# mdangschat/ctc-asr

Measured on AMD Instinct MI355X. Metric: audio-seconds/s training throughput (DS2, 10 s utterances), higher is better.
Workload: dtype f32 tensors / accumulate / own kernels; projection GEMMs: fp16x3 split (22 significand bits) where the layer input is bounded or, behind a ReLU cell, scaled per row / per column on the device - forward projections and their gradient GEMMs - bf16x6 split (24 bits) elsewhere; forward and backward recu

## Files before the change

ctc_asr_amd/csrc/rnn_persistent.hip:

```cpp
#include "common.h"
#include <stddef.h>
#include <stdlib.h>
#include <string.h>
#include <type_traits>
#include <vector>

#define PRNN_THREADS 256
#define PRNN_BLOCK_ROWS 32
#ifndef PRNN_GROUPS
#define PRNN_GROUPS 8
#endif
#define PRNN_SPIN_LIMIT (1u << 22)
#ifndef PRNN_PROBE_RS_Q
#define PRNN_PROBE_RS_Q 4
#endif
#ifndef PRNN_PROBE_HALF_LOADS
#define PRNN_PROBE_HALF_LOADS 0
#endif
#ifndef PRNN_XCD_AWARE
#define PRNN_XCD_AWARE 0
#endif
#ifndef PRNN_CHAIN_LB
#define PRNN_CHAIN_LB 4
#endif
// ... 41 lines not shown
    const float *b_hh;
    float *drec;
    float *dbias;
    int T, B, H, nwg;
    int BS;
    int ndir, dir0;
    int chain0;
    int s_lo, s_hi;
    float *carry;
    float *rs;
    unsigned *colmax;
    int prof;
    unsigned ticket;
    int xcd_split;
    unsigned *kp;
};

__device__ __forceinline__ float4 ldg4(const float *p) {
    return *reinterpret_cast<const float4 *>(p);
}
__device__ __forceinline__ void mma4(f32x4 &acc, const float4 &a, const float4 &b) {
    acc = __builtin_amdgcn_mfma_f32_16x16x4f32(a.x, b.x, acc, 0, 0, 0);
    acc = __builtin_amdgcn_mfma_f32_16x16x4f32(a.y, b.y, acc, 0, 0, 0);
    acc = __builtin_amdgcn_mfma_f32_16x16x4f32(a.z, b.z, acc, 0, 0, 0);
    acc = __builtin_amdgcn_mfma_f32_16x16x4f32(a.w, b.w, acc, 0, 0, 0);
}
__device__ __forceinline__ void mma4x2(f32x4 &acc0, f32x4 &acc1, const float4 &a0,
                                       const float4 &b0, const float4 &a1, const float4 &b1) {
    acc0 = __builtin_amdgcn_mfma_f32_16x16x4f32(a0.x, b0.x, acc0, 0, 0, 0);
    acc1 = __builtin_amdgcn_mfma_f32_16x16x4f32(a1.x, b1.x, acc1, 0, 0, 0);
// ... 482 lines not shown
                                         unsigned uniform_off) {
    return __builtin_amdgcn_raw_buffer_load_b128(rsrc, (int)lane_off, (int)uniform_off, 0);
}
template <int CTRL>
__device__ __forceinline__ unsigned dpp_u32(unsigned v) {
    return (unsigned)__builtin_amdgcn_update_dpp(0, (int)v, CTRL, 0xF, 0xF, false);
}
__device__ __forceinline__ void gather8_pieces(unsigned q0, u32x4 &first, u32x4 &second) {
    const unsigned q1 = dpp_u32<0x101>(q0), q2 = dpp_u32<0x102>(q0), q3 = dpp_u32<0x103>(q0),
                   q4 = dpp_u32<0x104>(q0), q5 = dpp_u32<0x105>(q0), q6 = dpp_u32<0x106>(q0),
                   q7 = dpp_u32<0x107>(q0);
    first = (u32x4){(q0 & 0xFFFFu) | (q1 << 16), (q2 & 0xFFFFu) | (q3 << 16),
                    (q4 & 0xFFFFu) | (q5 << 16), (q6 & 0xFFFFu) | (q7 << 16)};
    second = (u32x4){(q0 >> 16) | (q1 & 0xFFFF0000u), (q2 >> 16) | (q3 & 0xFFFF0000u),
                     (q4 >> 16) | (q5 & 0xFFFF0000u), (q6 >> 16) | (q7 & 0xFFFF0000u)};
}

template <int CELL, int NT, int KC, int REGW = 0>
__global__ void __launch_bounds__(PRNN_THREADS) prnn_fwd16_kernel(PArgs p) {
    constexpr bool GRU = CELL == CTCASR_CELL_GRU;
    constexpr int G = 4;
    constexpr int GR = GRU ? 3 : G;
    constexpr int COLS = 16 * NT;
    constexpr int UPB = COLS / G;
    constexpr int QS = KC * NT * 2;
    constexpr int QL = QS - REGW;
    constexpr int QW = 2 * KC;
    static_assert(16 * UPB <= PRNN_THREADS, "one item per thread");
    extern __shared__ __attribute__((aligned(16))) char smem[];
    resident_signal(p.sync, p.ticket);
// ... 1206 lines not shown
#ifndef PRNN_B16S_XCD_EXCL
#define PRNN_B16S_XCD_EXCL 0
#endif
#ifndef PRNN_B16S_JA
#define PRNN_B16S_JA 1
#endif
template <int DD, int JW, int JP, int JA, bool PROF = false>
__global__ void __launch_bounds__(PRNN_THREADS) prnn_bwd16s_kernel(PArgs p) {
    constexpr int H = PRNN_RS_H, GH = 4 * H;
    constexpr int NW = 4, NTH = 256, NPW = 16, QS = NPW * 4, QL = QS / 2, REGW = QS - QL;
    constexpr int RED_FLOATS = NW * 16 * 17, IVL = 4 * NPW;
    static_assert(DD % 2 == 0 && DD <= NPW && (NPW % DD == 0 || JW == NPW / 2 - 1),
                  "ring slots: even; not a divisor of 16 only when the next phase is requested at the end");
    static_assert(2 * JW >= NPW - DD && JW < NPW / 2 && JP <= JW && JA <= JP, "pipeline points");
    extern __shared__ __attribute__((aligned(16))) char smem[];
    resident_signal(p.sync, p.ticket);
    if (launch_poisoned(p.sync)) return;
    u32x4 *frag = reinterpret_cast<u32x4 *>(smem);
    float *red = reinterpret_cast<float *>(smem + (size_t)NW * QL * 64 * sizeof(u32x4));
    float4 *invs = reinterpret_cast<float4 *>(red + 2 * RED_FLOATS);
    float *wave_top = reinterpret_cast<float *>(invs + 2 * NW * IVL);
    unsigned *arrived = reinterpret_cast<unsigned *>(wave_top + 4);

    const int tid = threadIdx.x, lane = tid & 63;
    const int wave = __builtin_amdgcn_readfirstlane(tid >> 6);
#if PRNN_B16S_XCD_EXCL
    if (((int)blockIdx.x & 7) >= 4) return;
    const int dir = p.dir0 + (((int)blockIdx.x & 7) >> 1);
    const int slice = ((int)blockIdx.x >> 3) * 2 + ((int)blockIdx.x & 1);
#else
    const int wg = blockIdx.x % (p.ndir * p.nwg);
    const bool split = p.xcd_split && p.ndir == 2;
    const int dir = p.dir0 + (split ? (wg & 7) >> 2 : wg / p.nwg);
    const int slice = split ? (wg >> 3) * 4 + (wg & 3) : wg % p.nwg;
#endif
    const int group_size = p.nwg / PRNN_GROUPS, grp = slice / group_size;
    const int B = p.B, T = p.T, BS = p.BS;
    const int u0 = slice * 16;
    if (tid < 2) arrived[tid] = 0u;

    float w_scale;
    {
        float m = 0.f;
        const float *wrow = p.w + ((size_t)dir * H + u0 + (tid & 15)) * GH;
        for (int n = (tid >> 4) * 4; n < GH; n += NTH / 16 * 4) {
            const float4 v = ldg4(wrow + n);
            m = fmaxf(fmaxf(m, fmaxf(fabsf(v.x), fabsf(v.y))), fmaxf(fabsf(v.z), fabsf(v.w)));
        }
        m = wave_max(m);
        if (lane == 0) wave_top[wave] = m;
        __syncthreads();
        m = fmaxf(fmaxf(wave_top[0], wave_top[1]), fmaxf(wave_top[2], wave_top[3]));
        const unsigned bits = __float_as_uint(m);
        const int e = (int)((bits >> 23) & 0xFF) - 127;
        const int se = bits == 0u ? 0 : min(max(14 - e, -60), 60);
        w_scale = __uint_as_float((unsigned)(se + 127) << 23);
    }
    const float out_scale = 1.0f / w_scale;
    u32x4 wreg[REGW];
    {
        auto pieces = [&](int pm, u32x4 &first, u32x4 &second) {
            const float *wcol = p.w + ((size_t)dir * H + u0 + (lane & 15)) * GH +
                                16 * (wave * NPW + (pm >> 1)) + 8 * (pm & 1) + 2 * (lane >> 4);
            unsigned q[8];
#pragma unroll
            for (int e = 0; e < 8; ++e)
                q[e] = f16_pieces(wcol[(size_t)(e & 3) * H + (e >> 2)] * w_scale);
            first = (u32x4){(q[0] & 0xFFFFu) | (q[1] << 16), (q[2] & 0xFFFFu) | (q[3] << 16),
                            (q[4] & 0xFFFFu) | (q[5] << 16), (q[6] & 0xFFFFu) | (q[7] << 16)};
            second = (u32x4){(q[0] >> 16) | (q[1] & 0xFFFF0000u), (q[2] >> 16) | (q[3] & 0xFFFF0000u),
                             (q[4] >> 16) | (q[5] & 0xFFFF0000u), (q[6] >> 16) | (q[7] & 0xFFFF0000u)};
        };
        for (int pm = 0; pm < QL / 2; ++pm) {
            u32x4 first, second;
            pieces(pm, first, second);
            frag[(wave * QL + 2 * pm) * 64 + lane] = first;
            frag[(wave * QL + 2 * pm + 1) * 64 + lane] = second;
        }
#pragma unroll
        for (int pm = 0; pm < REGW / 2; ++pm) pieces(QL / 2 + pm, wreg[2 * pm], wreg[2 * pm + 1]);
    }
    __syncthreads();

    const __amdgpu_buffer_rsrc_t x_rsrc = __builtin_amdgcn_make_buffer_rsrc(
        p.xchg, 0, (int)((size_t)(T + 1) * 2 * B * GH * sizeof(float)), 0x00020000);
    const size_t x_step = (size_t)2 * B * GH;
    const size_t x_base = x_step;
    const __amdgpu_buffer_rsrc_t s_rsrc = __builtin_amdgcn_make_buffer_rsrc(
        p.rs, 0, (int)prnn_b16_scale_bytes(T), 0x00020000);
    constexpr unsigned S_STEP = 2u * (H / 16) * PRNN_B16_SCALE_ROWS * sizeof(float);
    const int rnum = 0x7FFFFFFF;
    const __amdgpu_buffer_rsrc_t dy_rsrc = __builtin_amdgcn_make_buffer_rsrc(
        const_cast<float *>(p.dy), 0, rnum, 0x00020000);
    const __amdgpu_buffer_rsrc_t g_rsrc = __builtin_amdgcn_make_buffer_rsrc(p.gates, 0, rnum, 0x00020000);
    const __amdgpu_buffer_rsrc_t c_rsrc = __builtin_amdgcn_make_buffer_rsrc(p.cells, 0, rnum, 0x00020000);
    const __amdgpu_buffer_rsrc_t dx_rsrc = __builtin_amdgcn_make_buffer_rsrc(p.dxw, 0, rnum, 0x00020000);
    auto ldf = [](__amdgpu_buffer_rsrc_t r, unsigned off) -> float {
// ... 1611 lines not shown
    }
    return CTCASR_ERR_BAD_ARGUMENT;
}

static size_t prnn_step_exchange_bytes(int T, int B, int H, int G) {
    return ctcasr_align_up((size_t)(T + 1) * 2 * B * G * H * sizeof(float), 256);
}
size_t prnn_exchange_bytes(int T, int B, int H, int G) {
    return prnn_step_exchange_bytes(T, B, H, G) +
           (G == 4 && H == PRNN_RS_H
                ? prnn_rs_ring_bytes() + ctcasr_align_up(prnn_b16_scale_bytes(T), 256) : 0) +
           (G == 4 && H == PRNN_W16_H ? ctcasr_align_up(prnn_w16_scale_bytes(T), 256) : 0) +
           (G == 1 && H == PRNN_R16_H ? prnn_r16_scale_bytes(T) : 0);
}

int prnn_fwd(int cell, const float *xw, const float *xw_bias, const float *w_hh,
             const float *b_hh_n, const int32_t *seq_len, int T, int B, int BS, int H, float *y,
             void *y16, float *gates, float *cells, void *sync, void *xchg, float *carry,
             int step_begin, int step_end, int flags, hipStream_t s) {
    const bool fwd_half_chip = (flags & CTCASR_RNN_HALF_CHIP) != 0;
    PArgs p = {};
    p.carry = carry;
    p.xchg = reinterpret_cast<float *>(xchg);
    p.xw = xw; p.w = w_hh; p.seq_len = seq_len; p.y = y; p.gates = gates; p.cells = cells;
    p.y16 = reinterpret_cast<unsigned short *>(y16);
    p.bias = xw_bias; p.b_hh = b_hh_n;
    p.ndir = 2; p.dir0 = 0; p.chain0 = 0;
    p.sync = reinterpret_cast<SyncWords *>(sync);
    p.T = T; p.B = B; p.BS = BS; p.H = H;
    p.s_lo = step_begin; p.s_hi = step_end;
// ... 78 lines not shown
        PRNN_FWD(CTCASR_CELL_LSTM, 2, 16, 2);
    }
    if (cell == CTCASR_CELL_RNN_RELU) {
        if (mt == 1) { PRNN_FWD(CTCASR_CELL_RNN_RELU, 1, 32, 1); }
        PRNN_FWD(CTCASR_CELL_RNN_RELU, 1, 32, 2);
    }
    if (mt == 1) { PRNN_FWD(CTCASR_CELL_RNN_TANH, 1, 32, 1); }
    PRNN_FWD(CTCASR_CELL_RNN_TANH, 1, 32, 2);
#undef PRNN_FWD
}

int prnn_bwd(int cell, const float *dy, const float *y, const float *w_hh_t,
             const int32_t *seq_len, int T, int B, int BS, int H, const float *gates,
             const float *cells, float *dxw, float *drec, float *dbias, unsigned *colmax,
             void *sync, void *kp, void *xchg, float *carry, int step_begin, int step_end,
             int flags, hipStream_t s) {
    PArgs p = {};
    p.dbias = dbias;
    p.s_lo = step_begin; p.s_hi = step_end; p.carry = carry;
    p.xchg = reinterpret_cast<float *>(xchg);
    p.w = w_hh_t; p.seq_len = seq_len; p.y = const_cast<float *>(y); p.dy = dy; p.dxw = dxw;
    p.drec = drec;
    p.gates = const_cast<float *>(gates); p.cells = const_cast<float *>(cells);
    p.sync = reinterpret_cast<SyncWords *>(sync);
    const bool half_chip = (flags & CTCASR_RNN_WHOLE_CHIP) == 0;
    p.T = T; p.B = B; p.BS = BS; p.H = H;
    p.ndir = 2; p.dir0 = 0; p.chain0 = 0;
    p.nwg = cell == CTCASR_CELL_LSTM ? (half_chip ? H / 16 : H / 8) : (half_chip ? H / 32 : H / 16);
    p.prof = getenv("CTCASR_RNN_PROF") != nullptr;
    p.ticket = ((unsigned)flags >> 8) & 0xFFFFFFu;
    p.xcd_split = (flags & CTCASR_RNN_XCD_SPLIT) != 0;
    const int mt = (B + 15) / 16;
    const bool chains = mt == 2 && !(flags & CTCASR_RNN_ONE_BARRIER);
// ... 187 lines not shown
```

ctc_asr_amd/csrc/rnn_step.hip:

```cpp
#include "common.h"

#define RNN_THREADS 256

namespace {

struct StepArgs {
    const float *xw;
    const float *w;
    const int *seq_len;
    float *y;
    const float *dy;
    float *dxw;
    float *gates;
    float *cells;
    float *hbuf;
    float *cbuf;
    const float *b_hh;
    const float *xw_bias;
    float *drec;
    int T, B, H, step;
};

__device__ __forceinline__ float4 ldg4(const float *p) {
    return *reinterpret_cast<const float4 *>(p);
// ... 227 lines not shown

extern "C" int ctcasr_rnn_persistent_supported(int cell, int T, int B, int H);
size_t prnn_sync_bytes();
size_t prnn_error_offset();
size_t prnn_kp_region_bytes(int H, int G);
int prnn_resident_gate(void *sync, unsigned ticket, int max_wait_us, hipStream_t s);
size_t prnn_exchange_bytes(int T, int B, int H, int G);
int prnn_fwd(int cell, const float *xw, const float *xw_bias, const float *w_hh,
             const float *b_hh_n, const int32_t *seq_len, int T, int B, int BS, int H, float *y,
             void *y16, float *gates, float *cells, void *sync, void *xchg, float *carry,
             int step_begin, int step_end, int flags, hipStream_t s);
int prnn_bwd(int cell, const float *dy, const float *y, const float *w_hh_t,
             const int32_t *seq_len, int T, int B, int BS, int H, const float *gates,
             const float *cells, float *dxw, float *drec, float *dbias, unsigned *colmax,
             void *sync, void *kp, void *xchg, float *carry, int step_begin, int step_end,
             int flags, hipStream_t s);

#define PRNN_BLOCK_ROWS 32
static int prnn_blocks(int B) { return (B + PRNN_BLOCK_ROWS - 1) / PRNN_BLOCK_ROWS; }
static int prnn_block_rows(int B, int block) {
    const int left = B - block * PRNN_BLOCK_ROWS;
    return left < PRNN_BLOCK_ROWS ? left : PRNN_BLOCK_ROWS;
}

static size_t rnn_state_bytes(int B, int H) {
    return ctcasr_align_up((size_t)6 * B * H * sizeof(float), 256);
}

static size_t prnn_ctl_bytes(int H, int G) {
    return ctcasr_align_up(prnn_sync_bytes(), 256) +
           ctcasr_align_up(prnn_kp_region_bytes(H, G), 256);
// ... 135 lines not shown
    const int rows = B < PRNN_BLOCK_ROWS ? B : PRNN_BLOCK_ROWS;
    return (flags & CTCASR_RNN_F16) &&
           ((cell == CTCASR_CELL_LSTM && (H == 1024 || H == 2048)) ||
            (cell == CTCASR_CELL_RNN_RELU && H == 2048 && rows <= 16 && B <= 16)) &&
           ctcasr_rnn_persistent_supported(cell, T, B, H) ? 1 : 0;
}

extern "C" int ctcasr_rnn_f16_recurrence(int cell, int T, int B, int H, int flags, int backward,
                                         int ragged) {
    if (cell == CTCASR_CELL_RNN_RELU)
        return !ragged && ctcasr_rnn_bwd_f16_supported(cell, T, B, H, flags);
    return backward ? ctcasr_rnn_bwd_f16_supported(cell, T, B, H, flags)
                    : ctcasr_rnn_fwd_f16_supported(cell, T, B, H, flags);
}

extern "C" int ctcasr_rnn_bwd_steps(int cell, const float *dy, const float *y,
                                    const float *w_hh_t, const float *b_hh_n,
                                    const int32_t *seq_len, int T, int B, int H,
                                    const void *reserve, float *dxw, float *dbias,
                                    uint32_t *colmax, void *workspace, size_t workspace_bytes,
                                    int step_begin, int step_end, int flags,
                                    ctcasr_stream_t stream) {
    (void)b_hh_n;
    if (colmax && (!ctcasr_rnn_bwd_f16_supported(cell, T, B, H, flags) ||
                   (cell == CTCASR_CELL_RNN_RELU && seq_len)))
        return CTCASR_ERR_UNSUPPORTED;
    int rc = rnn_check(cell, T, B, H);
    if (rc != CTCASR_OK) return rc;
    if (flags & 0xFF & ~(CTCASR_RNN_HALF_CHIP | CTCASR_RNN_WHOLE_CHIP | CTCASR_RNN_ONE_BARRIER |
                         CTCASR_RNN_REDUCE_SCATTER | CTCASR_RNN_F16 | CTCASR_RNN_XCD_SPLIT |
                         CTCASR_RNN_STAGGER | CTCASR_RNN_KPAIR))
        return CTCASR_ERR_BAD_ARGUMENT;
    if (!dy || !y || !w_hh_t || !reserve || !dxw) return CTCASR_ERR_BAD_ARGUMENT;
    if (step_begin < 0 || step_end > T || step_begin >= step_end) return CTCASR_ERR_BAD_ARGUMENT;
    if (!workspace || workspace_bytes < ctcasr_rnn_workspace_bytes(cell, T, B, H))
        return CTCASR_ERR_WORKSPACE;
    hipStream_t s = (hipStream_t)stream;
// ... 11 lines not shown
        return CTCASR_ERR_LAUNCH;
    if (cell == CTCASR_CELL_GRU && seq_len && step_end == T &&
        hipMemsetAsync(p.drec, 0, (size_t)T * B * 2 * G * H * sizeof(float), s) != hipSuccess)
        return CTCASR_ERR_LAUNCH;
    if (ctcasr_rnn_persistent_supported(cell, T, B, H)) {
        for (int blk = 0; blk < prnn_blocks(B); ++blk) {
            const size_t b0 = (size_t)blk * PRNN_BLOCK_ROWS;
            const PrnnBlock wb = prnn_block(workspace, T, B, H, G, blk);
            if (step_end == T &&
                (rc = prnn_clear_zero_block(wb, blk, prnn_block_rows(B, blk), H, G, s)) != CTCASR_OK)
                return rc;
            rc = prnn_bwd(cell, dy + b0 * 2 * H, y + b0 * 2 * H, w_hh_t,
                          seq_len ? seq_len + b0 : nullptr, T, prnn_block_rows(B, blk), B, H,
                          p.gates + b0 * 2 * 4 * H, p.cells + b0 * 2 * H, dxw + b0 * 2 * G * H,
                          p.drec + b0 * 2 * G * H, dbias, colmax, wb.sync, wb.kp, wb.xchg,
                          p.cbuf + b0 * 2 * H, step_begin, step_end, flags, s);
            if (rc != CTCASR_OK) return rc;
        }
        return CTCASR_OK;
    }
    dim3 grid(H / 16, 2, (B + 15) / 16);
    for (int step = step_end - 1; step >= step_begin; --step) {
        p.step = step;
        if (cell == CTCASR_CELL_LSTM)
            rnn_bwd_step_kernel<CTCASR_CELL_LSTM><<<grid, RNN_THREADS, 0, s>>>(p);
        else if (cell == CTCASR_CELL_GRU)
            rnn_bwd_step_kernel<CTCASR_CELL_GRU><<<grid, RNN_THREADS, 0, s>>>(p);
        else if (cell == CTCASR_CELL_RNN_RELU)
            rnn_bwd_step_kernel<CTCASR_CELL_RNN_RELU><<<grid, RNN_THREADS, 0, s>>>(p);
        else
            rnn_bwd_step_kernel<CTCASR_CELL_RNN_TANH><<<grid, RNN_THREADS, 0, s>>>(p);
    }
    if (ctcasr_launch_status() != CTCASR_OK) return CTCASR_ERR_LAUNCH;
    if (dbias && step_begin == 0) {
        rc = ctcasr_colsum_accumulate(dxw, dbias, (int64_t)T * B, 2 * G * H, stream);
        if (rc == CTCASR_OK && cell == CTCASR_CELL_GRU)
            rc = ctcasr_colsum_accumulate(p.drec, dbias + (size_t)2 * G * H, (int64_t)T * B,
                                          2 * G * H, stream);
        return rc;
    }
    return CTCASR_OK;
}

extern "C" int ctcasr_rnn_bwd(int cell, const float *dy, const float *y, const float *w_hh_t,
                              const float *b_hh_n, const int32_t *seq_len, int T, int B, int H,
                              const void *reserve, float *dxw, float *dbias, void *workspace,
                              size_t workspace_bytes, ctcasr_stream_t stream) {
    return ctcasr_rnn_bwd_steps(cell, dy, y, w_hh_t, b_hh_n, seq_len, T, B, H, reserve, dxw,
                                dbias, nullptr, workspace, workspace_bytes, 0, T,
                                CTCASR_RNN_DEFAULT, stream);
}

extern "C" size_t ctcasr_rnn_timeout_word_offset(int cell, int T, int B, int H, int block) {
    if (rnn_check(cell, T, B, H) != CTCASR_OK || !ctcasr_rnn_persistent_supported(cell, T, B, H) ||
        block < 0 || block >= prnn_blocks(B))
        return (size_t)-1;
// ... 42 lines not shown
```

ctc_asr_amd/hip.py:

```python

import ctypes
import functools
import os

import torch

_PKG_DIR = os.path.dirname(os.path.abspath(__file__))
LIB_PATH = os.path.join(_PKG_DIR, 'libctcasr.so')

ABI_VERSION = 7
BUILD_PROBE_WRONG_RESULTS, BUILD_NONDEFAULT_TUNING = 1, 2
RNN_DEFAULT, RNN_HALF_CHIP, RNN_WHOLE_CHIP, RNN_ONE_BARRIER = 0, 1, 2, 4
RNN_REDUCE_SCATTER = 8
RNN_F16 = 16
RNN_XCD_SPLIT = 32
RNN_STAGGER = 64
RNN_KPAIR = 128
GRAD_NORM_CHUNK = 8192
GRAD_NORM_MAX_SEGMENTS = 64
SPEC_AUGMENT_MAX_MASKS = 16
NOISE_MIX_CHUNK = 8192
NOISE_MIX_SNR_DB = (-20, 60)
REVERB_CHUNK = 2048
REVERB_TAP_BLOCK = 32
# ... 35 lines not shown
    'ctcasr_rnn_reserve_bytes': (_c_sz, [_c_int] * 4),
    'ctcasr_rnn_workspace_bytes': (_c_sz, [_c_int] * 4),
    'ctcasr_rnn_persistent_supported': (_c_int, [_c_int] * 4),
    'ctcasr_rnn_poll_error': (_c_int, [_c_p, _c_sz] + [_c_int] * 4 + [_c_p]),
    'ctcasr_rnn_resident_gate': (_c_int, [_c_p, _c_sz] + [_c_int] * 4 + [ctypes.c_uint, _c_int,
                                                                          _c_p]),
    'ctcasr_rnn_gru_drec_offset': (_c_sz, [_c_int] * 3),
    'ctcasr_rnn_fwd': (_c_int, [_c_int] + [_c_p] * 5 + [_c_int] * 3 + [_c_p] * 3 + [_c_sz, _c_p]),
    'ctcasr_rnn_bwd': (_c_int, [_c_int] + [_c_p] * 5 + [_c_int] * 3 + [_c_p] * 4 + [_c_sz, _c_p]),
    'ctcasr_rnn_fwd_steps': (_c_int, [_c_int] + [_c_p] * 5 + [_c_int] * 3 + [_c_p] * 4 +
                             [_c_sz, _c_int, _c_int, _c_int, _c_p]),
    'ctcasr_rnn_fwd_f16_supported': (_c_int, [_c_int] * 5),
    'ctcasr_rnn_bwd_steps': (_c_int, [_c_int] + [_c_p] * 5 + [_c_int] * 3 + [_c_p] * 5 +
                             [_c_sz, _c_int, _c_int, _c_int, _c_p]),
    'ctcasr_rnn_bwd_f16_supported': (_c_int, [_c_int] * 5),
    'ctcasr_bias_act_fwd': (_c_int, [_c_p, _c_p, _c_i64, _c_int, _c_f, _c_f, _c_u64, _c_p]),
    'ctcasr_bias_act_bwd': (_c_int, [_c_p] * 4 + [_c_i64, _c_int, _c_f, _c_f, _c_p]),
    'ctcasr_dropout': (_c_int, [_c_p, _c_p, _c_i64, _c_f, _c_u64, _c_p]),
    'ctcasr_colsum_accumulate': (_c_int, [_c_p, _c_p, _c_i64, _c_int, _c_p]),
    'ctcasr_conv_s12_supported': (_c_int, [_c_int, _c_int]),
    'ctcasr_conv_s12_pack_weights': (_c_int, [_c_p, _c_p, _c_int, _c_p]),
    'ctcasr_conv_s12_fwd': (_c_int, [_c_p, _c_p, _c_p, _c_p] + [_c_int] * 4 + [_c_f, _c_int, _c_p]),
    'ctcasr_conv_s12_pack16_bytes': (_c_sz, [_c_int]),
    'ctcasr_conv_s12_pack_weights16': (_c_int, [_c_p, _c_p, _c_int, _c_p]),
    'ctcasr_conv_s12_fwd16': (_c_int, [_c_p, _c_f, _c_p, _c_p, _c_p] + [_c_int] * 4 +
                              [_c_f, _c_int, _c_p]),
    'ctcasr_conv_s12_bwd_data16': (_c_int, [_c_p, _c_p, _c_p] + [_c_int] * 5 + [_c_p, _c_f, _c_p]),
    'ctcasr_conv0_pack16_bytes': (_c_sz, []),
    'ctcasr_conv0_pack_weights16': (_c_int, [_c_p, _c_p, _c_p]),
    'ctcasr_conv0_fwd16': (_c_int, [_c_p] * 4 + [_c_int, _c_int, _c_f, _c_p]),
# ... 532 lines not shown
        workspace = rnn_workspace(cell, num_steps, batch, hidden, dev)
    with _Timed('rnn_fwd'):
      _check(load().ctcasr_rnn_fwd_steps(
        CELL_IDS[cell], _dev(xw, name='xw'), _dev(xw_bias, name='xw_bias'),
        _dev(w_hh, name='w_hh'), _dev(b_hh_n, name='b_hh_n'),
        _dev(seq_len, torch.int32, 'seq_len'), num_steps, batch, hidden, _dev(y, name='y'),
        _dev(y16, torch.float16, 'y16'),
        _dev(reserve, torch.uint8, 'reserve'), _dev(workspace, torch.uint8, 'workspace'),
        workspace.numel(), int(begin), int(end), int(flags) | (int(ticket) & 0xFFFFFF) << 8,
        _stream()), 'rnn_fwd')
    return y, reserve, workspace


@_on_tensor_device
def rnn_bwd(cell, dy, y, w_hh_t, reserve, seq_len=None, b_hh_n=None, dxw=None, dbias=None,
            workspace=None, steps=None, flags=RNN_DEFAULT, ticket=0, colmax=None):
    num_steps, batch = dy.shape[0], dy.shape[1]
    hidden = w_hh_t.shape[1]
    gates = CELL_GATES[cell]
    dev = dy.device
    begin, end = (0, num_steps) if steps is None else steps
    if (begin, end) != (0, num_steps) and (dxw is None or workspace is None):
        raise ValueError('rnn_bwd: a partial step range needs the caller\'s dxw and workspace '
                         '(they carry the pass from one call to the next).')
    dxw = torch.empty((num_steps, batch, 2, gates * hidden), dtype=torch.float32, device=dev) \
        if dxw is None else dxw
    if workspace is None:
        workspace = rnn_workspace(cell, num_steps, batch, hidden, dev)
    with _Timed('rnn_bwd'):
      _check(load().ctcasr_rnn_bwd_steps(
        CELL_IDS[cell], _dev(dy, name='dy'), _dev(y, name='y'), _dev(w_hh_t, name='w_hh_t'),
        _dev(b_hh_n, name='b_hh_n'), _dev(seq_len, torch.int32, 'seq_len'), num_steps, batch,
        hidden, _dev(reserve, torch.uint8, 'reserve'), _dev(dxw, name='dxw'),
        _dev(dbias, name='dbias'), _dev(colmax, torch.int32, 'colmax'),
        _dev(workspace, torch.uint8, 'workspace'),
        workspace.numel(), int(begin), int(end), int(flags) | (int(ticket) & 0xFFFFFF) << 8,
        _stream()), 'rnn_bwd')
    return dxw


def rnn_fwd_f16_supported(cell, num_steps, batch, hidden, flags=RNN_F16):
    return bool(load().ctcasr_rnn_fwd_f16_supported(CELL_IDS[cell], int(num_steps), int(batch),
                                                    int(hidden), int(flags)))


def rnn_f16_recurrence(cell, num_steps, batch, hidden, flags=RNN_F16, backward=False,
                       ragged=False):
    return bool(load().ctcasr_rnn_f16_recurrence(CELL_IDS[cell], int(num_steps), int(batch),
                                                 int(hidden), int(flags), int(backward),
                                                 int(ragged)))


def rnn_bwd_f16_supported(cell, num_steps, batch, hidden, flags=RNN_F16):
# ... 1016 lines not shown
```

ctc_asr_amd/model.py:

```python

import contextlib
import math
import os

import numpy as np
import torch

from ctc_asr_amd import hip, metrics, split_gemm
from ctc_asr_amd.labels import num_classes
from ctc_asr_amd.params import ema_alpha_at

CONV_KERNEL_SIZES = ((11, 41), (11, 21), (11, 21))
CONV_STRIDES = ((2, 2), (1, 2), (1, 2))
GATES = {'lstm': 4, 'gru': 3, 'rnn_relu': 1, 'rnn_tanh': 1}


class InfeasibleAlignmentError(ValueError):
    """Raised where ``tf.nn.ctc_loss`` raises InvalidArgumentError ("Not enough time for target
    transition sequence"), ``ignore_longer_outputs_than_inputs=False`` (``asr/model.py:259``)."""


class ModelConfig:

    def __init__(self, used_model='ds2', conv_filters=(32, 32, 96), num_units_dense=2048,
# ... 332 lines not shown
        self.own_wgrad_parts = int(os.environ.get('CTCASR_WGRAD_PARTS', '2'))
        self.unbounded_f16 = os.environ.get('CTCASR_UNBOUNDED_F16', '1') == '1'
        self.dgrad_early = os.environ.get('CTCASR_DGRAD_EARLY', '0')
        self._dgrad_stream = None
        self.rnn_fwd_f16 = os.environ.get('CTCASR_RNN_FWD_F16', '1') == '1'
        self.rnn_bwd_f16 = os.environ.get('CTCASR_RNN_BWD_F16', '1') == '1'
        self.rnn_xcd_flag = hip.RNN_XCD_SPLIT \
            if os.environ.get('CTCASR_RNN_XCD_SPLIT', '1') == '1' else 0
        self.rnn_stagger_flag = hip.RNN_STAGGER \
            if os.environ.get('CTCASR_RNN_STAGGER', '1') == '1' else 0
        if os.environ.get('CTCASR_RNN_KPAIR', '0') == '1':
            self.rnn_stagger_flag |= hip.RNN_KPAIR
        self.rnn_kpair_wide = os.environ.get('CTCASR_RNN_KPAIR_2048', '1') == '1'
        self.rnn_fwd_pieces = os.environ.get('CTCASR_RNN_FWD_PIECES', '1') == '1'
        self._w_split, self._w_split_ready, self._w_split_bufs = {}, None, {}
        self._w_guard = None
        self._side_stream = None
        self.early_hooks = False
        self.rnn_bwd_flags = int(os.environ.get('CTCASR_RNN_BWD_FLAGS', str(hip.RNN_DEFAULT)))
        self.gpu_metrics = os.environ.get('CTCASR_GPU_METRICS', '1') == '1'
        self._rnn_ws = {}
        self.dropout_seed = int(seed) * 0x9E3779B1 + 1
        self._acts = None
        self._w_hh_t = [torch.empty((2, cfg.num_units_rnn, GATES[cfg.cell] * cfg.num_units_rnn),
                                    dtype=torch.float32, device=self.device)
                        for _ in range(cfg.num_layers_rnn)]

    def _upcoming_ticket(self):
        return self._ticket % 0xFFFFFF + 1

# ... 136 lines not shown
                    pieces.fwd16 = stacked16.view(-1, k4.shape[1])
                else:
                    pieces.make_fwd(buf('dense4/bf16', lambda: torch.empty(
                        (6,) + tuple(k4.shape), dtype=torch.bfloat16, device=self.device)))
                if training and dense4_f16 and self.bwd_f16:
                    pieces.tr16 = split_gemm.split16(
                        k4, split_gemm.W_SCALE, split_gemm.H_B,
                        out=buf('dense4/t16', lambda: split_gemm.empty16(
                            k4.shape[0], k4.shape[1], split_gemm.H_B, self.device)))
                elif training:
                    pieces.make_tr(buf('dense4/tbf16', lambda: split_gemm.empty(
                        k4.shape[0], k4.shape[1], split_gemm.A_ORDER, self.device)), None)
                self._w_split['dense4'] = pieces
            self._w_split_ready = torch.cuda.Event()
            self._w_split_ready.record(side)

    def _weight_split(self, name, backward=False, acts=None):
        pieces, ready = (self._w_split, self._w_split_ready) if acts is None else \
            (acts['w_split'], acts['w_split_ready'])
        got = pieces.get(name)
        if got is None:
            return None
        if ready is not None:
            torch.cuda.current_stream(self.device).wait_event(ready)
        return got

    def _next_seed(self):
        self.dropout_seed = (self.dropout_seed * 6364136223846793005 + 1442695040888963407) \
            & 0xFFFFFFFFFFFFFFFF
        return self.dropout_seed
# ... 174 lines not shown
                    rnn_len, b_hh_n=p['rnn{}/b_hh'.format(i)] if cell == 'gru' else None,
                    workspace=workspace, xw_bias=self._rnn_bias(i), flags=rnn_flags,
                    y16=None if y16 is None else y16.buf)
                y16_of = None if y16 is None else (y, y16, split_gemm.RNN_F16_H_SCALE)
            arithmetic['rnn{}/recurrence_fwd'.format(i)] = rnn_form
            layer_in.append(x)
            layer_out.append(y)
            reserves.append(reserve)
            x = y
            in_bound = None if cell == 'rnn_relu' else 1.0
            if rnn_rate > 0.0 and not cfg.cudnn:
                seeds[1] = self._next_seed()
                x = hip.dropout(x, rnn_rate, seeds[1])
                in_bound = in_bound / (1.0 - rnn_rate) if in_bound is not None else None
            drop_seeds.append(seeds)
        acts.update(layer_in=layer_in, layer_out=layer_out, reserves=reserves, rnn_ws=workspace,
                    rnn_len=rnn_len, t_out=t_out, drop_seeds=drop_seeds, rnn_rate=rnn_rate,
                    in_split=in_split, out_split=[None] * cfg.num_layers_rnn,
                    in_split16=in_split16)

        rnn_flat = x.view(t_out * batch, 2 * hidden)
        flat_split, k4_pieces = None, self._weight_split('dense4')
        acts['flat16'] = None
        flat_scale = split_gemm.f16_scale(in_bound) \
            if k4_pieces is not None and k4_pieces[2] is not None else None
        if flat_scale is None and k4_pieces is not None and k4_pieces[2] is not None and \
                k4_pieces.rows_form:
            acts['flat16'] = split_gemm.ColScaled(rnn_flat)
            dense4 = split_gemm.mm_rows16(rnn_flat, k4_pieces[2], split_gemm.W_SCALE,
                                          stacked=True)
# ... 470 lines not shown
                      acts['rnn_len'] is None and
                      hip.dgrad16_supported(cell, t_out, batch, hidden))
            early_dg = own_dg and chunks > 1 and self.dgrad_early in ('side', 'own') and \
                side is not main
            dx2d, dg_done = None, []
            if early_dg:
                dx2d = torch.zeros((rows, w_ih.shape[1]), dtype=torch.float32, device=dy.device)
                side_tensors.append(dx2d)

            def dgrad_share(lo, hi, dx2d=dx2d, w_pieces=w_pieces, n=w_ih.shape[1]):
                for d, (a, b) in enumerate(((lo, hi), (t_out - hi, t_out - lo))):
                    hip.dgrad16_blockscaled(acts['rnn_ws'], t_out, batch, hidden, w_pieces.dg16,
                                            split_gemm.W_SCALE, n, out=dx2d, steps=(a, b),
                                            dirs=(d, d + 1), accumulate=True)

            for c in range(chunks):
                hip.rnn_bwd(cell, dy, y, self._w_hh_t[i], acts['reserves'][i], acts['rnn_len'],
                            dxw=dxw, dbias=dbias, workspace=acts['rnn_ws'],
                            steps=(bounds[c + 1], bounds[c]), flags=bwd_flags,
                            ticket=self._take_ticket() if persistent and not whole_chip_rnn
                            else 0, colmax=None if colmax is None else colmax[c])
                if c + 1 < chunks:
                    if early_dg and self.dgrad_early == 'own':
                        if self._dgrad_stream is None:
                            self._dgrad_stream = torch.cuda.Stream(self.device)
                        ready = torch.cuda.Event()
                        ready.record(main)
                        with torch.cuda.stream(self._dgrad_stream):
                            self._dgrad_stream.wait_event(ready)
                            if persistent:
                                self._gate_side_stream(cell, acts['rnn_ws'], t_out, batch, hidden)
                            dgrad_share(bounds[c + 1], bounds[c])
                            dg_done.append(torch.cuda.Event())
                            dg_done[-1].record(self._dgrad_stream)
                        dx2d.record_stream(self._dgrad_stream)

# ... 466 lines not shown
```

include/ctcasr.h:

```cpp
#ifndef CTCASR_H_
#define CTCASR_H_

#include <stddef.h>
#include <stdint.h>

#ifdef __cplusplus
extern "C" {
#endif

#define CTCASR_ABI_VERSION 7

enum {
    CTCASR_OK = 0,
    CTCASR_ERR_BAD_ARGUMENT = -1,
    CTCASR_ERR_UNSUPPORTED = -2,
    CTCASR_ERR_WORKSPACE = -3,
    CTCASR_ERR_LAUNCH = -4,
    CTCASR_ERR_TIMEOUT = -5
};

enum {
    CTCASR_CELL_RNN_RELU = 0,
    CTCASR_CELL_RNN_TANH = 1,
    CTCASR_CELL_LSTM = 2,
// ... 91 lines not shown
int ctcasr_rnn_poll_error(void *workspace, size_t workspace_bytes, int cell, int T, int B,
                          int H, ctcasr_stream_t stream);
int ctcasr_rnn_resident_gate(void *workspace, size_t workspace_bytes, int cell, int T, int B,
                             int H, unsigned ticket, int max_wait_us, ctcasr_stream_t stream);
int ctcasr_rnn_bwd(int cell, const float *dy, const float *y, const float *w_hh_t,
                   const float *b_hh_n, const int32_t *seq_len, int T, int B, int H,
                   const void *reserve, float *dxw, float *dbias, void *workspace,
                   size_t workspace_bytes, ctcasr_stream_t stream);
int ctcasr_rnn_bwd_steps(int cell, const float *dy, const float *y, const float *w_hh_t,
                         const float *b_hh_n, const int32_t *seq_len, int T, int B, int H,
                         const void *reserve, float *dxw, float *dbias, uint32_t *colmax,
                         void *workspace, size_t workspace_bytes, int step_begin, int step_end,
                         int flags, ctcasr_stream_t stream);
int ctcasr_rnn_bwd_f16_supported(int cell, int T, int B, int H, int flags);
int ctcasr_rnn_f16_recurrence(int cell, int T, int B, int H, int flags, int backward, int ragged);

int ctcasr_bias_act_fwd(float *y, const float *bias, int64_t rows, int cols, float cutoff,
                        float dropout_rate, uint64_t seed, ctcasr_stream_t stream);
int ctcasr_bias_act_bwd(const float *y, const float *dy, float *dz, float *dbias, int64_t rows,
                        int cols, float cutoff, float dropout_rate, ctcasr_stream_t stream);
int ctcasr_dropout(const float *in, float *out, int64_t n, float dropout_rate, uint64_t seed,
                   ctcasr_stream_t stream);
int ctcasr_colsum_accumulate(const float *dz, float *dbias, int64_t rows, int cols,
                             ctcasr_stream_t stream);

int ctcasr_conv_s12_supported(int freq_in, int cout);
int ctcasr_conv_s12_pack_weights(const float *w, float *packed, int cout, ctcasr_stream_t stream);
size_t ctcasr_conv_s12_pack16_bytes(int cout);
int ctcasr_conv_s12_pack_weights16(const float *w, void *packed16, int cout,
                                   ctcasr_stream_t stream);
// ... 161 lines not shown
```

Before: 6678.

## Prepack backward LSTM recurrent weights into f16 pieces on a side stream

New measurement: 6726, median of 3. Within noise of the previous version (+0.7%).

```diff
diff --git a/ctc_asr_amd/csrc/rnn_persistent.hip b/ctc_asr_amd/csrc/rnn_persistent.hip
--- a/ctc_asr_amd/csrc/rnn_persistent.hip
+++ b/ctc_asr_amd/csrc/rnn_persistent.hip
@@ -79,6 +79,7 @@
     unsigned ticket;
     int xcd_split;
     unsigned *kp;
+    const unsigned *wpack;
 };
 
 __device__ __forceinline__ float4 ldg4(const float *p) {
@@ -591,6 +592,107 @@
                     (q4 & 0xFFFFu) | (q5 << 16), (q6 & 0xFFFFu) | (q7 << 16)};
     second = (u32x4){(q0 >> 16) | (q1 & 0xFFFF0000u), (q2 >> 16) | (q3 & 0xFFFF0000u),
                      (q4 >> 16) | (q5 & 0xFFFF0000u), (q6 >> 16) | (q7 & 0xFFFF0000u)};
+}
+
+#define PRNN_WPACK_HEADER 256
+__host__ __device__ constexpr unsigned wpack_geometry(int backward, int cell, int H, int upb,
+                                                      int regw, int slices) {
+    return 0xA8000000u | (unsigned)backward << 26 | (unsigned)cell << 24 |
+           (unsigned)(H / 64) << 18 | (unsigned)upb << 12 | (unsigned)regw << 5 |
+           (unsigned)(slices / 32);
+}
+__host__ __device__ constexpr size_t wpack_scale_bytes(int slices) {
+    return ((size_t)2 * slices * sizeof(float) + 255) / 256 * 256;
+}
+__host__ __device__ constexpr size_t wpack_bytes(int slices, int qs) {
+    return PRNN_WPACK_HEADER + wpack_scale_bytes(slices) +
+           (size_t)2 * slices * 4 * qs * 64 * sizeof(u32x4);
+}
+__device__ __forceinline__ float wpack_pow2_scale(float m) {
+    const unsigned bits = __float_as_uint(m);
+    const int e = (int)((bits >> 23) & 0xFF) - 127;
+    const int se = bits == 0u ? 0 : min(max(14 - e, -60), 60);
+    return __uint_as_float((unsigned)(se + 127) << 23);
+}
+__device__ __forceinline__ void wpack_pieces(const float (&v)[8], float w_scale, u32x4 &first,
+                                             u32x4 &second) {
+    unsigned q[8];
+#pragma unroll
+    for (int e = 0; e < 8; ++e) q[e] = f16_pieces(v[e] * w_scale);
+    first = (u32x4){(q[0] & 0xFFFFu) | (q[1] << 16), (q[2] & 0xFFFFu) | (q[3] << 16),
+                    (q[4] & 0xFFFFu) | (q[5] << 16), (q[6] & 0xFFFFu) | (q[7] << 16)};
+    second = (u32x4){(q[0] >> 16) | (q[1] & 0xFFFF0000u), (q[2] >> 16) | (q[3] & 0xFFFF0000u),
+                     (q[4] >> 16) | (q[5] & 0xFFFF0000u), (q[6] >> 16) | (q[7] & 0xFFFF0000u)};
+}
+__global__ void __launch_bounds__(PRNN_THREADS) prnn_wpack_kernel(const float *w, unsigned *pack,
+                                                                  unsigned geometry, int H,
+                                                                  int slices) {
+    __shared__ float wave_top[4];
+    const int tid = threadIdx.x, lane = tid & 63, wave = tid >> 6;
+    const int dir = (int)blockIdx.x / slices, slice = (int)blockIdx.x % slices;
+    const int GH = 4 * H;
+    const int u0 = slice * 16;
+    const int pairs = (H / 64) * 2;
+    auto wload = [&](int pr, float (&v)[8]) {
+        const int n = 16 * (wave * (H / 64) + (pr >> 1)) + 8 * (pr & 1) + 2 * (lane >> 4);
+        const float *wcol = w + (size_t)dir * GH * H + u0 + (lane & 15);
+#pragma unroll
+        for (int e = 0; e < 8; ++e) v[e] = wcol[(size_t)((e & 3) * H + (e >> 2) + n) * H];
+    };
+    float m = 0.f;
+    for (int pr = 0; pr < pairs; ++pr) {
+        float v[8];
+        wload(pr, v);
+#pragma unroll
+        for (int e = 0; e < 8; ++e) m = fmaxf(m, fabsf(v[e]));
+    }
+    m = wave_max(m);
+    if (lane == 0) wave_top[wave] = m;
+    __syncthreads();
+    m = fmaxf(fmaxf(wave_top[0], wave_top[1]), fmaxf(wave_top[2], wave_top[3]));
+    const float w_scale = wpack_pow2_scale(m);
+    if (tid == 0) {
+        reinterpret_cast<float *>(pack + PRNN_WPACK_HEADER / 4)[dir * slices + slice] = w_scale;
+        if (blockIdx.x == 0) pack[0] = geometry;
+    }
+    u32x4 *out = reinterpret_cast<u32x4 *>(reinterpret_cast<char *>(pack) + PRNN_WPACK_HEADER +
+                                           wpack_scale_bytes(slices)) +
+                 ((size_t)blockIdx.x * 4 + wave) * (2 * pairs) * 64 + lane;
+    for (int pr = 0; pr < pairs; ++pr) {
+        float v[8];
+        wload(pr, v);
+        u32x4 first, second;
+        wpack_pieces(v, w_scale, first, second);
+        out[(size_t)(2 * pr) * 64] = first;
+        out[(size_t)(2 * pr + 1) * 64] = second;
+    }
+}
+__device__ __forceinline__ void wpack_dma16(const char *base, unsigned lane_off, unsigned lds_base) {
+    unsigned keep;
+    asm volatile("s_mov_b32 %0, m0\n\ts_mov_b32 m0, %3\n\ts_nop 0\n\t"
+                 "global_load_lds_dwordx4 %1, %2\n\ts_mov_b32 m0, %0"
+                 : "=&s"(keep)
+                 : "v"(lane_off), "s"(base), "s"(lds_base)
+                 : "memory");
+}
+template <int QL, int REGW, int NR>
+__device__ __forceinline__ float wpack_stage(const unsigned *wpack, int slices, int dir, int slice,
+                                             int wave, int lane, char *smem, u32x4 (&wreg)[NR]) {
+    constexpr int QS = QL + REGW;
+    const int uwave = __builtin_amdgcn_readfirstlane(wave);
+    const char *base = reinterpret_cast<const char *>(wpack) + PRNN_WPACK_HEADER;
+    const float w_scale = reinterpret_cast<const float *>(base)[dir * slices + slice];
+    const char *src = base + wpack_scale_bytes(slices) +
+                      ((size_t)(dir * slices + slice) * 4 + uwave) * QS * 1024;
+    const unsigned lds0 = __builtin_amdgcn_readfirstlane(
+        (unsigned)(uintptr_t)(__attribute__((address_space(3))) char *)smem) + uwave * QL * 1024;
+#pragma unroll
+    for (int q = 0; q < QL; ++q) wpack_dma16(src + q * 1024, lane * 16, lds0 + q * 1024);
+    const u32x4 *rsrc = reinterpret_cast<const u32x4 *>(src + QL * 1024) + lane;
+#pragma unroll
+    for (int q = 0; q < REGW; ++q) wreg[q] = rsrc[q * 64];
+    asm volatile("s_waitcnt vmcnt(0)" ::: "memory");
+    return w_scale;
 }
 
 template <int CELL, int NT, int KC, int REGW = 0>
@@ -1827,6 +1929,7 @@
                   "ring slots: even; not a divisor of 16 only when the next phase is requested at the end");
     static_assert(2 * JW >= NPW - DD && JW < NPW / 2 && JP <= JW && JA <= JP, "pipeline points");
     extern __shared__ __attribute__((aligned(16))) char smem[];
+    const unsigned long long t_entry = PROF ? wall_clock64() : 0;
     resident_signal(p.sync, p.ticket);
     if (launch_poisoned(p.sync)) return;
     u32x4 *frag = reinterpret_cast<u32x4 *>(smem);
@@ -1853,6 +1956,12 @@
     if (tid < 2) arrived[tid] = 0u;
 
     float w_scale;
+    u32x4 wreg[REGW];
+    const bool packed = p.wpack &&
+                        p.wpack[0] == wpack_geometry(1, CTCASR_CELL_LSTM, H, 16, REGW, p.nwg);
+    if (packed) {
+        w_scale = wpack_stage<QL, REGW>(p.wpack, p.nwg, dir, slice, wave, lane, smem, wreg);
+    } else {
     {
         float m = 0.f;
         const float *wrow = p.w + ((size_t)dir * H + u0 + (tid & 15)) * GH;
@@ -1869,8 +1978,6 @@
         const int se = bits == 0u ? 0 : min(max(14 - e, -60), 60);
         w_scale = __uint_as_float((unsigned)(se + 127) << 23);
     }
-    const float out_scale = 1.0f / w_scale;
-    u32x4 wreg[REGW];
     {
         auto pieces = [&](int pm, u32x4 &first, u32x4 &second) {
             const float *wcol = p.w + ((size_t)dir * H + u0 + (lane & 15)) * GH +
@@ -1893,7 +2000,10 @@
 #pragma unroll
         for (int pm = 0; pm < REGW / 2; ++pm) pieces(QL / 2 + pm, wreg[2 * pm], wreg[2 * pm + 1]);
     }
+    }
+    const float out_scale = 1.0f / w_scale;
     __syncthreads();
+    if (PROF && tid == 0 && blockIdx.x == 0) p.sync->prof[13] = wall_clock64() - t_entry;
 
     const __amdgpu_buffer_rsrc_t x_rsrc = __builtin_amdgcn_make_buffer_rsrc(
         p.xchg, 0, (int)((size_t)(T + 1) * 2 * B * GH * sizeof(float)), 0x00020000);
@@ -3535,6 +3645,45 @@
            (G == 1 && H == PRNN_R16_H ? prnn_r16_scale_bytes(T) : 0);
 }
 
+struct WpackGeom { int slices, qs, upb, regw; };
+static bool wpack_geom(int cell, int B, int H, int flags, int backward, WpackGeom *g) {
+    if (!backward || cell != CTCASR_CELL_LSTM || H != PRNN_RS_H || !(flags & CTCASR_RNN_F16))
+        return false;
+    const int rows = B < PRNN_BLOCK_ROWS ? B : PRNN_BLOCK_ROWS, mt = (rows + 15) / 16;
+    const bool half_chip = (flags & CTCASR_RNN_WHOLE_CHIP) == 0;
+    if (mt != 2 || !half_chip || rows % 8 != 0 || (flags & CTCASR_RNN_KPAIR) ||
+        !(flags & CTCASR_RNN_STAGGER))
+        return false;
+    *g = {PRNN_RS_NWG, 64, 16, 32};
+    return true;
+}
+static const unsigned *wpack_usable(int cell, int B, int H, int flags, int backward,
+                                    const void *wpack, size_t wpack_bytes_given) {
+    WpackGeom g;
+    if (!wpack || !wpack_geom(cell, B, H, flags, backward, &g) ||
+        wpack_bytes_given < wpack_bytes(g.slices, g.qs))
+        return nullptr;
+    return reinterpret_cast<const unsigned *>(wpack);
+}
+
+extern "C" size_t ctcasr_rnn_wpack_bytes(int cell, int B, int H, int flags, int backward) {
+    WpackGeom g;
+    return wpack_geom(cell, B, H, flags, backward, &g) ? wpack_bytes(g.slices, g.qs) : 0;
+}
+
+extern "C" int ctcasr_rnn_wpack(int cell, const float *w_hh, int B, int H, int flags, int backward,
+                                void *pack, size_t pack_bytes, ctcasr_stream_t stream) {
+    WpackGeom g;
+    if (!wpack_geom(cell, B, H, flags, backward, &g)) return CTCASR_ERR_UNSUPPORTED;
+    if (!w_hh || !pack || (reinterpret_cast<uintptr_t>(pack) & 15)) return CTCASR_ERR_BAD_ARGUMENT;
+    if (pack_bytes < wpack_bytes(g.slices, g.qs)) return CTCASR_ERR_WORKSPACE;
+    const unsigned geometry = wpack_geometry(backward ? 1 : 0, cell, H, g.upb, g.regw, g.slices);
+    hipStream_t s = (hipStream_t)stream;
+    prnn_wpack_kernel<<<2 * g.slices, PRNN_THREADS, 0, s>>>(
+        w_hh, reinterpret_cast<unsigned *>(pack), geometry, H, g.slices);
+    return ctcasr_launch_status();
+}
+
 int prnn_fwd(int cell, const float *xw, const float *xw_bias, const float *w_hh,
              const float *b_hh_n, const int32_t *seq_len, int T, int B, int BS, int H, float *y,
              void *y16, float *gates, float *cells, void *sync, void *xchg, float *carry,
@@ -3643,9 +3792,10 @@
              const int32_t *seq_len, int T, int B, int BS, int H, const float *gates,
              const float *cells, float *dxw, float *drec, float *dbias, unsigned *colmax,
              void *sync, void *kp, void *xchg, float *carry, int step_begin, int step_end,
-             int flags, hipStream_t s) {
+             int flags, const void *wpack, size_t wpack_bytes_given, hipStream_t s) {
     PArgs p = {};
     p.dbias = dbias;
+    p.wpack = wpack_usable(cell, B, H, flags, 1, wpack, wpack_bytes_given);
     p.s_lo = step_begin; p.s_hi = step_end; p.carry = carry;
     p.xchg = reinterpret_cast<float *>(xchg);
     p.w = w_hh_t; p.seq_len = seq_len; p.y = const_cast<float *>(y); p.dy = dy; p.dxw = dxw;
diff --git a/ctc_asr_amd/csrc/rnn_step.hip b/ctc_asr_amd/csrc/rnn_step.hip
--- a/ctc_asr_amd/csrc/rnn_step.hip
+++ b/ctc_asr_amd/csrc/rnn_step.hip
@@ -265,7 +265,7 @@
              const int32_t *seq_len, int T, int B, int BS, int H, const float *gates,
              const float *cells, float *dxw, float *drec, float *dbias, unsigned *colmax,
              void *sync, void *kp, void *xchg, float *carry, int step_begin, int step_end,
-             int flags, hipStream_t s);
+             int flags, const void *wpack, size_t wpack_bytes, hipStream_t s);
 
 #define PRNN_BLOCK_ROWS 32
 static int prnn_blocks(int B) { return (B + PRNN_BLOCK_ROWS - 1) / PRNN_BLOCK_ROWS; }
@@ -431,13 +431,14 @@
                     : ctcasr_rnn_fwd_f16_supported(cell, T, B, H, flags);
 }
 
-extern "C" int ctcasr_rnn_bwd_steps(int cell, const float *dy, const float *y,
-                                    const float *w_hh_t, const float *b_hh_n,
-                                    const int32_t *seq_len, int T, int B, int H,
-                                    const void *reserve, float *dxw, float *dbias,
-                                    uint32_t *colmax, void *workspace, size_t workspace_bytes,
-                                    int step_begin, int step_end, int flags,
-                                    ctcasr_stream_t stream) {
+extern "C" int ctcasr_rnn_bwd_steps_wp(int cell, const float *dy, const float *y,
+                                       const float *w_hh_t, const float *b_hh_n,
+                                       const int32_t *seq_len, int T, int B, int H,
+                                       const void *reserve, float *dxw, float *dbias,
+                                       uint32_t *colmax, void *workspace, size_t workspace_bytes,
+                                       int step_begin, int step_end, int flags,
+                                       const void *wpack, size_t wpack_bytes,
+                                       ctcasr_stream_t stream) {
     (void)b_hh_n;
     if (colmax && (!ctcasr_rnn_bwd_f16_supported(cell, T, B, H, flags) ||
                    (cell == CTCASR_CELL_RNN_RELU && seq_len)))
@@ -479,7 +480,7 @@
                           seq_len ? seq_len + b0 : nullptr, T, prnn_block_rows(B, blk), B, H,
                           p.gates + b0 * 2 * 4 * H, p.cells + b0 * 2 * H, dxw + b0 * 2 * G * H,
                           p.drec + b0 * 2 * G * H, dbias, colmax, wb.sync, wb.kp, wb.xchg,
-                          p.cbuf + b0 * 2 * H, step_begin, step_end, flags, s);
+                          p.cbuf + b0 * 2 * H, step_begin, step_end, flags, wpack, wpack_bytes, s);
             if (rc != CTCASR_OK) return rc;
         }
         return CTCASR_OK;
@@ -505,6 +506,18 @@
         return rc;
     }
     return CTCASR_OK;
+}
+
+extern "C" int ctcasr_rnn_bwd_steps(int cell, const float *dy, const float *y,
+                                    const float *w_hh_t, const float *b_hh_n,
+                                    const int32_t *seq_len, int T, int B, int H,
+                                    const void *reserve, float *dxw, float *dbias,
+                                    uint32_t *colmax, void *workspace, size_t workspace_bytes,
+                                    int step_begin, int step_end, int flags,
+                                    ctcasr_stream_t stream) {
+    return ctcasr_rnn_bwd_steps_wp(cell, dy, y, w_hh_t, b_hh_n, seq_len, T, B, H, reserve, dxw,
+                                   dbias, colmax, workspace, workspace_bytes, step_begin, step_end,
+                                   flags, nullptr, 0, stream);
 }
 
 extern "C" int ctcasr_rnn_bwd(int cell, const float *dy, const float *y, const float *w_hh_t,
diff --git a/ctc_asr_amd/hip.py b/ctc_asr_amd/hip.py
--- a/ctc_asr_amd/hip.py
+++ b/ctc_asr_amd/hip.py
@@ -73,6 +73,10 @@
     'ctcasr_rnn_bwd_steps': (_c_int, [_c_int] + [_c_p] * 5 + [_c_int] * 3 + [_c_p] * 5 +
                              [_c_sz, _c_int, _c_int, _c_int, _c_p]),
     'ctcasr_rnn_bwd_f16_supported': (_c_int, [_c_int] * 5),
+    'ctcasr_rnn_wpack_bytes': (_c_sz, [_c_int] * 5),
+    'ctcasr_rnn_wpack': (_c_int, [_c_int, _c_p] + [_c_int] * 4 + [_c_p, _c_sz, _c_p]),
+    'ctcasr_rnn_bwd_steps_wp': (_c_int, [_c_int] + [_c_p] * 5 + [_c_int] * 3 + [_c_p] * 5 +
+                                [_c_sz, _c_int, _c_int, _c_int, _c_p, _c_sz, _c_p]),
     'ctcasr_bias_act_fwd': (_c_int, [_c_p, _c_p, _c_i64, _c_int, _c_f, _c_f, _c_u64, _c_p]),
     'ctcasr_bias_act_bwd': (_c_int, [_c_p] * 4 + [_c_i64, _c_int, _c_f, _c_f, _c_p]),
     'ctcasr_dropout': (_c_int, [_c_p, _c_p, _c_i64, _c_f, _c_u64, _c_p]),
@@ -635,7 +639,7 @@
 
 @_on_tensor_device
 def rnn_bwd(cell, dy, y, w_hh_t, reserve, seq_len=None, b_hh_n=None, dxw=None, dbias=None,
-            workspace=None, steps=None, flags=RNN_DEFAULT, ticket=0, colmax=None):
+            workspace=None, steps=None, flags=RNN_DEFAULT, ticket=0, colmax=None, wpack=None):
     num_steps, batch = dy.shape[0], dy.shape[1]
     hidden = w_hh_t.shape[1]
     gates = CELL_GATES[cell]
@@ -649,15 +653,35 @@
     if workspace is None:
         workspace = rnn_workspace(cell, num_steps, batch, hidden, dev)
     with _Timed('rnn_bwd'):
-      _check(load().ctcasr_rnn_bwd_steps(
+      _check(load().ctcasr_rnn_bwd_steps_wp(
         CELL_IDS[cell], _dev(dy, name='dy'), _dev(y, name='y'), _dev(w_hh_t, name='w_hh_t'),
         _dev(b_hh_n, name='b_hh_n'), _dev(seq_len, torch.int32, 'seq_len'), num_steps, batch,
         hidden, _dev(reserve, torch.uint8, 'reserve'), _dev(dxw, name='dxw'),
         _dev(dbias, name='dbias'), _dev(colmax, torch.int32, 'colmax'),
         _dev(workspace, torch.uint8, 'workspace'),
         workspace.numel(), int(begin), int(end), int(flags) | (int(ticket) & 0xFFFFFF) << 8,
+        _dev(wpack, torch.uint8, 'wpack'), 0 if wpack is None else wpack.numel(),
         _stream()), 'rnn_bwd')
     return dxw
+
+
+def rnn_wpack_bytes(cell, batch, hidden, flags=RNN_F16 | RNN_STAGGER, backward=True):
+    return load().ctcasr_rnn_wpack_bytes(CELL_IDS[cell], int(batch), int(hidden), int(flags),
+                                         int(bool(backward)))
+
+
+@_on_tensor_device
+def rnn_wpack(cell, w_hh, batch, flags=RNN_F16 | RNN_STAGGER, backward=True, out=None):
+    hidden = w_hh.shape[2]
+    need = rnn_wpack_bytes(cell, batch, hidden, flags, backward)
+    if need == 0:
+        raise CtcAsrError('rnn_wpack: this launch takes no weight pack.')
+    out = torch.empty(need, dtype=torch.uint8, device=w_hh.device) if out is None else out
+    _expect_numel('rnn_wpack', 'w_hh', w_hh, 2 * 4 * hidden * hidden)
+    _check(load().ctcasr_rnn_wpack(CELL_IDS[cell], _dev(w_hh, name='w_hh'), int(batch), hidden,
+                                   int(flags), int(bool(backward)), _dev(out, torch.uint8, 'out'),
+                                   out.numel(), _stream()), 'rnn_wpack')
+    return out
 
 
 def rnn_fwd_f16_supported(cell, num_steps, batch, hidden, flags=RNN_F16):
diff --git a/ctc_asr_amd/model.py b/ctc_asr_amd/model.py
--- a/ctc_asr_amd/model.py
+++ b/ctc_asr_amd/model.py
@@ -370,6 +370,8 @@
         self.rnn_kpair_wide = os.environ.get('CTCASR_RNN_KPAIR_2048', '1') == '1'
         self.rnn_fwd_pieces = os.environ.get('CTCASR_RNN_FWD_PIECES', '1') == '1'
         self._w_split, self._w_split_ready, self._w_split_bufs = {}, None, {}
+        self.rnn_wpack = os.environ.get('CTCASR_RNN_WPACK', '1') == '1'
+        self._wpack = {}
         self._w_guard = None
         self._side_stream = None
         self.early_hooks = False
@@ -536,6 +538,57 @@
                 self._w_split['dense4'] = pieces
             self._w_split_ready = torch.cuda.Event()
             self._w_split_ready.record(side)
+
+    def _wpack_tag(self):
+        return (self.arena.version, self.step_count)
+
+    def _rnn_wpack_flags(self):
+        if not self.rnn_bwd_f16:
+            return None
+        return self.rnn_bwd_flags | hip.RNN_F16 | self.rnn_xcd_flag | self.rnn_stagger_flag
+
+    def _prepare_rnn_wpacks(self, rows, training, batch):
+        cfg = self.cfg
+        if not (training and self.rnn_wpack and batch and cfg.cell == 'lstm' and
+                rows % batch == 0 and
+                hip.rnn_persistent_supported(cfg.cell, rows // batch, batch, cfg.num_units_rnn)):
+            return
+        hidden, tag, flags = cfg.num_units_rnn, self._wpack_tag(), self._rnn_wpack_flags()
+        nbytes = 0 if flags is None else hip.rnn_wpack_bytes(cfg.cell, batch, hidden, flags)
+        if nbytes == 0:
+            return
+        key = (min(batch, 32), flags, nbytes)
+        todo = [i for i in reversed(range(cfg.num_layers_rnn))
+                if self._wpack.get(i) is None or self._wpack[i]['key'] != key or
+                self._wpack[i]['tag'] != tag]
+        if not todo:
+            return
+        main = torch.cuda.current_stream(self.device)
+        if self._side_stream is None:
+            self._side_stream = torch.cuda.Stream(self.device)
+        side = self._side_stream
+        start = torch.cuda.Event()
+        start.record(main)
+        side.wait_event(start)
+        with torch.cuda.stream(side):
+            for i in todo:
+                have = self._wpack.get(i)
+                buf = have['buf'] if have is not None and have['buf'].numel() >= nbytes else \
+                    torch.empty(nbytes, dtype=torch.uint8, device=self.device)
+                hip.rnn_wpack(cfg.cell, self.arena.p['rnn{}/w_hh'.format(i)], batch, flags,
+                              out=buf)
+                ready = torch.cuda.Event()
+                ready.record(side)
+                self._wpack[i] = {'buf': buf, 'key': key, 'tag': tag, 'ready': ready}
+
+    def _rnn_wpack_for(self, layer, batch, flags):
+        have = self._wpack.get(layer) if self.rnn_wpack else None
+        if have is None or have['tag'] != self._wpack_tag() or \
+                have['key'][:2] != (min(batch, 32), flags):
+            return None
+        if have['ready'] is not None:
+            torch.cuda.current_stream(self.device).wait_event(have['ready'])
+        return have['buf']
 
     def _weight_split(self, name, backward=False, acts=None):
         pieces, ready = (self._w_split, self._w_split_ready) if acts is None else \
@@ -740,6 +793,7 @@
                 x = hip.dropout(x, rnn_rate, seeds[1])
                 in_bound = in_bound / (1.0 - rnn_rate) if in_bound is not None else None
             drop_seeds.append(seeds)
+        self._prepare_rnn_wpacks(t_out * batch, training, batch)
         acts.update(layer_in=layer_in, layer_out=layer_out, reserves=reserves, rnn_ws=workspace,
                     rnn_len=rnn_len, t_out=t_out, drop_seeds=drop_seeds, rnn_rate=rnn_rate,
                     in_split=in_split, out_split=[None] * cfg.num_layers_rnn,
@@ -1240,12 +1294,13 @@
                                             split_gemm.W_SCALE, n, out=dx2d, steps=(a, b),
                                             dirs=(d, d + 1), accumulate=True)
 
+            wpack = self._rnn_wpack_for(i, batch, bwd_flags)
             for c in range(chunks):
                 hip.rnn_bwd(cell, dy, y, self._w_hh_t[i], acts['reserves'][i], acts['rnn_len'],
                             dxw=dxw, dbias=dbias, workspace=acts['rnn_ws'],
                             steps=(bounds[c + 1], bounds[c]), flags=bwd_flags,
                             ticket=self._take_ticket() if persistent and not whole_chip_rnn
-                            else 0, colmax=None if colmax is None else colmax[c])
+                            else 0, colmax=None if colmax is None else colmax[c], wpack=wpack)
                 if c + 1 < chunks:
                     if early_dg and self.dgrad_early == 'own':
                         if self._dgrad_stream is None:
diff --git a/include/ctcasr.h b/include/ctcasr.h
--- a/include/ctcasr.h
+++ b/include/ctcasr.h
@@ -129,6 +129,15 @@
                          int flags, ctcasr_stream_t stream);
 int ctcasr_rnn_bwd_f16_supported(int cell, int T, int B, int H, int flags);
 int ctcasr_rnn_f16_recurrence(int cell, int T, int B, int H, int flags, int backward, int ragged);
+size_t ctcasr_rnn_wpack_bytes(int cell, int B, int H, int flags, int backward);
+int ctcasr_rnn_wpack(int cell, const float *w_hh, int B, int H, int flags, int backward,
+                     void *pack, size_t pack_bytes, ctcasr_stream_t stream);
+int ctcasr_rnn_bwd_steps_wp(int cell, const float *dy, const float *y, const float *w_hh_t,
+                            const float *b_hh_n, const int32_t *seq_len, int T, int B, int H,
+                            const void *reserve, float *dxw, float *dbias, uint32_t *colmax,
+                            void *workspace, size_t workspace_bytes, int step_begin, int step_end,
+                            int flags, const void *wpack, size_t wpack_bytes,
+                            ctcasr_stream_t stream);
 
 int ctcasr_bias_act_fwd(float *y, const float *bias, int64_t rows, int cols, float cutoff,
                         float dropout_rate, uint64_t seed, ctcasr_stream_t stream);
```
